# NIH-NEI/oct-image-segmentation-models

Hardware: AMD Instinct MI355X
Metric: B-scans/sec (train step), 256x512 3-class U-Net (higher is better)
Workload: dtype f32; 1 GPU; configs[1]: train step (fwd+Dice-macro+bwd+allreduce+Adam), per-GPU batch 32, 256x512x1, 3-class, pool_layers=4, start_neurons=8, random-init weights; global_batch=32, parallelism=dp1, allreduce=none

## Files before the change

oct-image-segmentation-models_amd/csrc/kernels_bx.hpp:

```cpp
#pragma once
#include <type_traits>

#include "kernels_bwd.hpp"
#include "kernels_igemm.hpp"

namespace oct {

typedef __bf16 bf16x8 __attribute__((ext_vector_type(8)));

__device__ __forceinline__ uint32_t pk_bf16(float a, float b) {
    return __builtin_bit_cast(uint32_t, __builtin_convertvector(f32x2_hw{a, b}, bf16x2_hw));
}

__device__ __forceinline__ void touch_raw(float4& v) { asm volatile("" : "+v"(v.x), "+v"(v.y), "+v"(v.z), "+v"(v.w)); }
__device__ __forceinline__ void touch_raw(uint2& v) { asm volatile("" : "+v"(v.x), "+v"(v.y)); }

__device__ __forceinline__ void act8(float (&v)[8], const float (&fa)[8], const float (&fb)[8], float lo, bool in) {
    const float cl = in ? lo : 0.f, ch = in ? 3.0e38f : 0.f;
#pragma unroll
    for (int i = 0; i < 8; i += 2) {
        const f32x2_hw y = __builtin_elementwise_fma(f32x2_hw{fa[i], fa[i + 1]}, f32x2_hw{v[i], v[i + 1]}, f32x2_hw{fb[i], fb[i + 1]});
        v[i] = __builtin_amdgcn_fmed3f(y[0], cl, ch); v[i + 1] = __builtin_amdgcn_fmed3f(y[1], cl, ch);
    }
}
// ... 360 lines not shown
                    }
            }
        }
    };
    constexpr int EPN = EPI == EPI_MASK ? 4 * MB : (EPI == EPI_FWD ? MB : 0), EPF = (EPN + NTHR - 1) / NTHR;
    float epi_pf[EPF > 0 ? EPF : 1];
    auto load_epi = [&]() {
#pragma unroll
        for (int i = 0; i < EPF; ++i) {
            const int e = tid + i * NTHR;
            float v = 0.f;
            if constexpr (EPI == EPI_FWD) { if (e < MB && m0 + e < A.Mout) v = A.bias[A.m_off + m0 + e]; }
            else if constexpr (EPI == EPI_MASK) { if (e < 4 * MB && m0 + e % MB < A.Mout) v = A.bnin[(e / MB) * A.Mout + m0 + e % MB]; }
            epi_pf[i] = v;
        }
    };
    int g = 0;
#if defined(BX_DBG) && (BX_DBG == 6 || BX_DBG == 7)
    const int nch_run = 0;
    if constexpr (NW == 4) load_zraw();
    load_epi();
#if BX_DBG == 7
    if (A.Cin > 0) return;
#endif
#else
    const int nch_run = nch;
#endif
    for (int c = 0; c < nch_run; ++c) {
#pragma unroll
        for (int ky = 0; ky < KH; ++ky, ++g) {
            const bool last_row = ky == KH - 1, more = c + 1 < nch;
            if (last_row && !more) {
                if constexpr (NW == 4) load_zraw();
                load_epi();
            }
            if (last_row && more) {
#pragma unroll
                for (int k = 0; k < NSLOT; ++k) {
                    touch_raw(pin[k][0]); touch_raw(pin[k][1]);
                    if constexpr (GB) { touch_raw(pz[k][0]); touch_raw(pz[k][1]); }
                }
                if constexpr (NIMG == 2) begin_store((c + 1) * 16);
            }
#if !(defined(BX_DBG) && BX_DBG == 5)
            if (!last_row) dma_slab(c, ky + 1, (g + 1) & 1);
            else if (more) dma_slab(c + 1, 0, (g + 1) & 1);
#endif
            if (ky == 0 && more) load_in((c + 1) * 16);
            if constexpr (NIMG == 2) {
                if (last_row && more) sweep_row(ky, g & 1, c & 1, std::true_type{}, (c + 1) & 1);
                else sweep_row(ky, g & 1, c & 1, std::false_type{}, 0);
            } else {
                sweep_row(ky, g & 1, 0, std::false_type{}, 0);
                if (last_row && more) {
                    begin_store((c + 1) * 16);
                    __syncthreads();
#pragma unroll
                    for (int k = 0; k < NSLOT; ++k) store_slot(k, 0);
                }
            }
            asm volatile("s_waitcnt vmcnt(0)" ::: "memory");
#if !(defined(BX_DBG) && BX_DBG == 1)
            __syncthreads();
#endif
        }
    }
#if defined(BX_DBG) && BX_DBG == 1
    __syncthreads();
#endif

    float* const epi = reinterpret_cast<float*>(WTs);
    float* const red = reinterpret_cast<float*>(WTs + EPI_B);
    if constexpr (NW != 4) load_zraw();
    if constexpr (EPI != EPI_RAW) {
#pragma unroll
        for (int i = 0; i < EPF; ++i) { const int e = tid + i * NTHR; if (e < EPN) epi[e] = epi_pf[i]; }
    }
    __syncthreads();
    float s1[MTW][ACC], s2[MTW][ACC];
#pragma unroll
    for (int mt = 0; mt < MTW; ++mt)
#pragma unroll
        for (int r = 0; r < ACC; ++r) { s1[mt][r] = 0.f; s2[mt][r] = 0.f; }
#pragma unroll
    for (int nt = 0; nt < NTW; ++nt) {
        const int y = y0 + wave * NTW + nt, x = x0 + j;
        const bool pvalid = y < A.Ho && x < A.Wo;
        const size_t pix = pvalid ? ((size_t)b * A.Ho + y) * A.Wo + x : 0;
#pragma unroll
        for (int mt = 0; mt < MTW; ++mt) {
#pragma unroll
            for (int q = 0; q < QUADS; ++q) {
                const int ml = mt * MT + 8 * q + 4 * h, m = m0 + ml;
                const bool valid = pvalid && m < A.Mout;
                float v[4] = {acc[mt][nt][4 * q], acc[mt][nt][4 * q + 1], acc[mt][nt][4 * q + 2], acc[mt][nt][4 * q + 3]};
                if constexpr (EPI == EPI_FWD) {
                    if (valid) {
                        const float4 bs = ld4(epi + ml);
                        v[0] += bs.x; v[1] += bs.y; v[2] += bs.z; v[3] += bs.w;
                    }
#pragma unroll
                    for (int k = 0; k < 4; ++k) {
                        const float u = valid ? v[k] : 0.f;
                        s1[mt][4 * q + k] += u; s2[mt][4 * q + k] += u * u;
                    }
                } else if constexpr (EPI == EPI_MASK) {
                    const float4 zq = widen4(zraw[nt][mt][q]);
                    const float zz[4] = {zq.x, zq.y, zq.z, zq.w};
                    const float4 ea = ld4(epi + BN_A * MB + ml), eb = ld4(epi + BN_B * MB + ml);
                    const float4 em = ld4(epi + BN_MEAN * MB + ml), er = ld4(epi + BN_RSTD * MB + ml);
                    const float ka[4] = {ea.x, ea.y, ea.z, ea.w}, kb[4] = {eb.x, eb.y, eb.z, eb.w};
                    const float km[4] = {em.x, em.y, em.z, em.w}, kr[4] = {er.x, er.y, er.z, er.w};
#pragma unroll
                    for (int k = 0; k < 4; ++k) {
                        const int cc = valid ? m + k : 0;
                        const float yv = fmaf(ka[k], zz[k], kb[k]);
                        float gv = v[k];
                        if (A.drop_out) gv *= drop_mul(A.drop, (uint32_t)(pix * A.Mout + cc));
                        gv = (valid && yv > 0.f) ? gv : 0.f;
                        const float xh = (zz[k] - km[k]) * kr[k];
                        v[k] = gv; s1[mt][4 * q + k] += gv; s2[mt][4 * q + k] += gv * xh;
                    }
                }
                if (valid) sta4<AT>(reinterpret_cast<AT*>(A.out) + pix * A.Mout + m, make_float4(v[0], v[1], v[2], v[3]));
            }
        }
    }
    if constexpr (EPI != EPI_RAW) {
        if (A.part) {
#pragma unroll
            for (int mt = 0; mt < MTW; ++mt) {
                subgroup_reduce_rec<ACC, ACC, 16>(s1[mt], lane);
                subgroup_reduce_rec<ACC, ACC, 16>(s2[mt], lane);
                const int ci = sub_chan<ACC, 16>(lane);
                const int mloc = 8 * (ci >> 2) + 4 * h + (ci & 3);
                red[((wave * 2 + 0) * MTW + mt) * MT + mloc] = s1[mt][0];
                red[((wave * 2 + 1) * MTW + mt) * MT + mloc] = s2[mt][0];
            }
            __syncthreads();
            if (tid < 2 * MB) {
                const int stat = tid / MB, ml = tid % MB, mt = ml / MT, mloc = ml % MT;
                float s = 0.f;
#pragma unroll
                for (int w = 0; w < NW; ++w) s += red[((w * 2 + stat) * MTW + mt) * MT + mloc];
                if (m0 + ml < A.Mout)
                    A.part[((size_t)b * A.tiles + tile) * (2 * A.Mout) + (size_t)stat * A.Mout + m0 + ml] = s;
            }
        }
    }
}

typedef __bf16 bf16x4 __attribute__((ext_vector_type(4)));

template <int KH, bool UP, int NS, typename AT, bool DROP = false, bool GB = false>
__global__ __launch_bounds__(kBlock, 1) void conv_dwbx_k(const ConvBwdWArgs A) {
    constexpr int TH = 4, TW = 32, TAPS = KH * KH;
    constexpr int IH = UP ? TH + 1 : TH + KH - 1, IW = UP ? TW + 1 : TW + KH - 1, PT = UP ? 0 : (KH - 1) / 2;
    constexpr int NPX = IH * IW, NPD = TH * TW;
    constexpr int NXS = (NPX * 4 + kBlock - 1) / kBlock, NDS = (NPD * 4) / kBlock;
    constexpr int NPXP = NXS * (kBlock / 4);
    constexpr int XPL = NPXP * 64, DPL = NPD * 64;
    constexpr int BUF_B = NS * (XPL + DPL);
    static_assert((NPD * 4) % kBlock == 0, "dz tile items");
    constexpr int RED_B = TAPS * 4 * 16 * 64 * 4;
    constexpr int SMEM_B = 2 * BUF_B > RED_B ? 2 * BUF_B : RED_B;
    static_assert(SMEM_B >= 4096 * 4 + kBlock * 8 * 4, "bias scratch fits");
    __shared__ __attribute__((aligned(256))) char smem[SMEM_B];

    const int tid = threadIdx.x, lane = tid & 63, wave = __builtin_amdgcn_readfirstlane(tid >> 6);
    const int ci0 = blockIdx.y * 32, co0 = blockIdx.z * 32;
    const int Hs = UP ? A.H >> 1 : A.H, Ws = UP ? A.W >> 1 : A.W;

    const int o8 = 8 * (tid & 3);
    const int cx = ci0 + o8;
    const bool two = (A.flags & F_TWO) && cx >= A.C0;
    const int Cs = two ? A.C1 : A.C0, ccx = two ? cx - A.C0 : cx;
    const AT* __restrict__ xsrc = (two ? reinterpret_cast<const AT*>(A.x1) : reinterpret_cast<const AT*>(A.x0)) + ccx;
    const AT* __restrict__ dsrc = reinterpret_cast<const AT*>(A.dz) + co0 + o8;
    const AT* __restrict__ zsrc = GB ? reinterpret_cast<const AT*>(A.zf) + co0 + o8 : nullptr;
    const bool aff = (A.flags & F_AFF) != 0;
    const float lo = aff ? 0.f : -3.0e38f;
    float fa[8], fb[8];
#pragma unroll
    for (int i = 0; i < 8; ++i) { fa[i] = 1.f; fb[i] = 0.f; }
    if (aff) {
        const float* ab = two ? A.ab1 : A.ab0;
#pragma unroll
        for (int i = 0; i < 8; ++i) { fa[i] = ab[ccx + i]; fb[i] = ab[Cs + ccx + i]; }
    }
    float ga[GB ? 8 : 1], gb[GB ? 8 : 1], gd[GB ? 8 : 1];
    if constexpr (GB) load_gb8(A.bnf, A.Cout, co0 + o8, ga, gb, gd);
    int xly[NXS], xlx[NXS];
#pragma unroll
    for (int k = 0; k < NXS; ++k) {
        const int P = (tid >> 2) + k * (kBlock / 4);
        xly[k] = P < NPX ? P / IW : -1000000; xlx[k] = P % IW;
    }
    struct Regs { typename Raw4<AT>::type x[NXS][2], d[NDS][2], z[GB ? NDS : 1][2]; };
    float bsum[8];
#pragma unroll
    for (int i = 0; i < 8; ++i) bsum[i] = 0.f;

    auto tile_of = [&](int tl, int& b, int& y0, int& x0) {
        b = tl / A.tiles; const int t = tl % A.tiles;
        x0 = (t % A.tiles_x) * TW; y0 = (t / A.tiles_x) * TH;
    };
    struct Geo { int b, y0, x0; };
    auto geo_of = [&](int tl) { Geo g; tile_of(tl, g.b, g.y0, g.x0); return g; };
    auto load_item = [&](int i, const Geo& g, Regs& R) {
        if (i < NXS) {
            const int k = i;
            int gy = g.y0 + xly[k] - PT, gx = g.x0 + xlx[k] - PT;
            gy = gy < 0 ? 0 : (gy >= A.H ? A.H - 1 : gy); gx = gx < 0 ? 0 : (gx >= A.W ? A.W - 1 : gx);
            const int sy = UP ? gy >> 1 : gy, sx = UP ? gx >> 1 : gx;
            const AT* p = xsrc + (((size_t)g.b * Hs + sy) * Ws + sx) * Cs;
            R.x[k][0] = ldraw4<AT>(p); R.x[k][1] = ldraw4<AT>(p + 4);
        } else {
            const int k = i - NXS;
            const int P = (tid >> 2) + k * (kBlock / 4);
            int py = g.y0 + P / TW, px = g.x0 + P % TW;
            py = py >= A.H ? A.H - 1 : py; px = px >= A.W ? A.W - 1 : px;
            const size_t e = (((size_t)g.b * A.H + py) * A.W + px) * A.Cout;
            R.d[k][0] = ldraw4<AT>(dsrc + e); R.d[k][1] = ldraw4<AT>(dsrc + e + 4);
            if constexpr (GB) { R.z[k][0] = ldraw4<AT>(zsrc + e); R.z[k][1] = ldraw4<AT>(zsrc + e + 4); }
        }
    };
    auto store_item = [&](int i, const Geo& g, const Regs& R, int buf, bool live) {
        if (i < NXS) {
            const int k = i;
            const float4 v0 = widen4(R.x[k][0]), v1 = widen4(R.x[k][1]);
            float v[8] = {v0.x, v0.y, v0.z, v0.w, v1.x, v1.y, v1.z, v1.w};
            const int gy = g.y0 + xly[k] - PT, gx = g.x0 + xlx[k] - PT;
            const bool in = gy >= 0 && gy < A.H && gx >= 0 && gx < A.W;
            act8(v, fa, fb, lo, in);
            if constexpr (DROP) {
                const int sy = UP ? gy >> 1 : gy, sx = UP ? gx >> 1 : gx;
                const uint32_t el = (uint32_t)((((size_t)g.b * Hs + sy) * Ws + sx) * Cs + ccx);
#pragma unroll
                for (int e = 0; e < 8; ++e) v[e] = in ? v[e] * drop_mul(A.drop, el + e) : 0.f;
            }
            uint4 pl[NS];
            split8<NS>(v, pl);
            const int P = (tid >> 2) + k * (kBlock / 4);
            char* d = smem + buf * BUF_B + o8 * 2 + P * 64;
#pragma unroll
            for (int p = 0; p < NS; ++p) *reinterpret_cast<uint4*>(d + p * XPL) = pl[p];
        } else {
            const int k = i - NXS;
            const int P = (tid >> 2) + k * (kBlock / 4);
            const bool in = live && g.y0 + P / TW < A.H && g.x0 + P % TW < A.W;
            const float4 v0 = widen4(R.d[k][0]), v1 = widen4(R.d[k][1]);
            float v[8] = {v0.x, v0.y, v0.z, v0.w, v1.x, v1.y, v1.z, v1.w};
            if constexpr (GB) {
                const float4 z0 = widen4(R.z[k][0]), z1 = widen4(R.z[k][1]);
                const float zv[8] = {z0.x, z0.y, z0.z, z0.w, z1.x, z1.y, z1.z, z1.w};
                gb8<AT>(v, zv, ga, gb, gd, in);
#pragma unroll
                for (int e = 0; e < 8; ++e) bsum[e] += v[e];
            } else {
#pragma unroll
                for (int e = 0; e < 8; ++e) { v[e] = in ? v[e] : 0.f; bsum[e] += v[e]; }
            }
            uint4 pl[NS];
            split8<NS>(v, pl);
            char* d = smem + buf * BUF_B + NS * XPL + o8 * 2 + P * 64;
#pragma unroll
            for (int p = 0; p < NS; ++p) *reinterpret_cast<uint4*>(d + p * DPL) = pl[p];
        }
    };
    constexpr int NIT = NXS + NDS;
    auto load = [&](int tl, Regs& R) {
        const Geo g = geo_of(tl);
#pragma unroll
        for (int i = 0; i < NIT; ++i) load_item(i, g, R);
    };
    auto store = [&](int tl, const Regs& R, int buf, bool live) {
        const Geo g = geo_of(tl);
#pragma unroll
        for (int i = 0; i < NIT; ++i) store_item(i, g, R, buf, live);
    };

    f32x16 acc[TAPS];
#pragma unroll
    for (int t = 0; t < TAPS; ++t)
#pragma unroll
        for (int r = 0; r < 16; ++r) acc[t][r] = 0.f;

    const int laneoff = (8 * (lane >> 5) + ((lane & 15) >> 2)) * 64 + (16 * ((lane >> 4) & 1) + 4 * (lane & 3)) * 2;
    auto tr8 = [&](const char* base) -> bf16x8 {
        const bf16x4 lo = __builtin_amdgcn_ds_read_tr16_b64_v4bf16((__attribute__((address_space(3))) bf16x4*)(base));
        const bf16x4 hi = __builtin_amdgcn_ds_read_tr16_b64_v4bf16((__attribute__((address_space(3))) bf16x4*)(base + 4 * 64));
        return bf16x8{lo[0], lo[1], lo[2], lo[3], hi[0], hi[1], hi[2], hi[3]};
    };
    constexpr int KS = TW / 16, STEPS = KS * TAPS;
    auto compute = [&](int buf, auto&& between) {
        const char* Xl = smem + buf * BUF_B + laneoff;
        const char* Dl = smem + buf * BUF_B + NS * XPL + laneoff + (wave * TW) * 64;
        constexpr int DEPTH = 3;
        bf16x8 av[DEPTH][NS], bw[2][NS];
        auto fetch_a = [&](int st, bf16x8 (&f)[NS]) {
            const int ks = st / TAPS, t = st % TAPS, ky = t / KH, kx = t % KH;
#pragma unroll
            for (int p = 0; p < NS; ++p) f[p] = tr8(Xl + p * XPL + ((wave + ky) * IW + ks * 16 + kx) * 64);
        };
        auto fetch_b = [&](int ks, bf16x8 (&f)[NS]) {
#pragma unroll
            for (int p = 0; p < NS; ++p) f[p] = tr8(Dl + p * DPL + ks * 16 * 64);
        };
        __builtin_amdgcn_s_setprio(1);
        fetch_b(0, bw[0]); fetch_a(0, av[0]); fetch_a(1, av[1]);
#pragma unroll
        for (int st = 0; st < STEPS; ++st) {
            if (st + 2 < STEPS) fetch_a(st + 2, av[(st + 2) % DEPTH]);
            if (st % TAPS == TAPS - 2 && st / TAPS + 1 < KS) fetch_b(st / TAPS + 1, bw[(st / TAPS + 1) & 1]);
            const int t = st % TAPS;
            const bf16x8 (&a)[NS] = av[st % DEPTH];
            const bf16x8 (&bv)[NS] = bw[(st / TAPS) & 1];
            f32x16 c = acc[t];
            if constexpr (NS == 3) {
                c = __builtin_amdgcn_mfma_f32_32x32x16_bf16(a[0], bv[2], c, 0, 0, 0);
                c = __builtin_amdgcn_mfma_f32_32x32x16_bf16(a[2], bv[0], c, 0, 0, 0);
                c = __builtin_amdgcn_mfma_f32_32x32x16_bf16(a[1], bv[1], c, 0, 0, 0);
                c = __builtin_amdgcn_mfma_f32_32x32x16_bf16(a[0], bv[1], c, 0, 0, 0);
                c = __builtin_amdgcn_mfma_f32_32x32x16_bf16(a[1], bv[0], c, 0, 0, 0);
            }
            c = __builtin_amdgcn_mfma_f32_32x32x16_bf16(a[0], bv[0], c, 0, 0, 0);
            acc[t] = c;
            between(st);
        }
        __builtin_amdgcn_s_setprio(0);
        constexpr int NPROD = NS == 3 ? 6 : 1, RPF = 2 * NS;
        constexpr int VPS = NS == 3 ? (UP ? 40 : 26) : (UP ? 24 : 14);
        constexpr int WPS = NS;
        __builtin_amdgcn_sched_group_barrier(0x100, 3 * RPF, 0);
#pragma unroll
        for (int st = 0; st < STEPS; ++st) {
            if (st + 2 < STEPS) __builtin_amdgcn_sched_group_barrier(0x100, RPF, 0);
            if (st % TAPS == TAPS - 2 && st / TAPS + 1 < KS) __builtin_amdgcn_sched_group_barrier(0x100, RPF, 0);
            __builtin_amdgcn_sched_group_barrier(0x008, NPROD, 0);
            __builtin_amdgcn_sched_group_barrier(0x002, VPS, 0);
            if (((st + 1) * NIT) / STEPS != (st * NIT) / STEPS) {
                __builtin_amdgcn_sched_group_barrier(0x200, WPS, 0);
                if (GB && (st * NIT) / STEPS >= NXS) __builtin_amdgcn_sched_group_barrier(0x020, 4, 0);
                else __builtin_amdgcn_sched_group_barrier(0x020, 2, 0);
            }
        }
    };

    Regs R;
    const int t0 = blockIdx.x, step = A.npb, tend = A.total_tiles, tlast = tend - 1;
    if (t0 < tend) {
        load(t0, R);
        store(t0, R, 0, true);
        load(t0 + step < tend ? t0 + step : tlast, R);
    }
    __syncthreads();
    int buf = 0;
    for (int tl = t0; tl < tend; tl += step, buf ^= 1) {
        const int t1 = tl + step, t2 = tl + 2 * step;
        const Geo g1 = geo_of(t1 < tend ? t1 : tlast), g2 = geo_of(t2 < tend ? t2 : tlast);
        const bool live = t1 < tend;
        compute(buf, [&](int st) {
#pragma unroll
            for (int i = 0; i < NIT; ++i)
                if (((st + 1) * NIT) / STEPS != (st * NIT) / STEPS && (st * NIT) / STEPS == i) {
                    store_item(i, g1, R, buf ^ 1, live);
                    load_item(i, g2, R);
                }
        });
        __syncthreads();
    }

    float* const red = reinterpret_cast<float*>(smem);
    float4* const red4 = reinterpret_cast<float4*>(smem);
    const size_t wsize = (size_t)TAPS * A.Cin * A.Cout;
    float* out = A.part + (size_t)blockIdx.x * (wsize + A.Cout);
    __syncthreads();
#pragma unroll
    for (int t = 0; t < TAPS; ++t)
#pragma unroll
        for (int q = 0; q < 4; ++q)
            red4[((wave * TAPS + t) * 4 + q) * 64 + lane] = make_float4(acc[t][4 * q], acc[t][4 * q + 1], acc[t][4 * q + 2], acc[t][4 * q + 3]);
    __syncthreads();
#pragma unroll
    for (int t = 0; t < TAPS; ++t) {
        const int q = wave, e = (t * 4 + q) * 64 + lane;
        const float4 w0 = red4[e], w1 = red4[TAPS * 256 + e], w2 = red4[2 * TAPS * 256 + e], w3 = red4[3 * TAPS * 256 + e];
        const float sv[4] = {(w0.x + w1.x) + (w2.x + w3.x), (w0.y + w1.y) + (w2.y + w3.y),
                             (w0.z + w1.z) + (w2.z + w3.z), (w0.w + w1.w) + (w2.w + w3.w)};
        const int col = lane & 31, row0 = 8 * q + 4 * (lane >> 5);
#pragma unroll
        for (int jr = 0; jr < 4; ++jr)
            if (ci0 + row0 + jr < A.Cin && co0 + col < A.Cout)
                out[((size_t)t * A.Cin + ci0 + row0 + jr) * A.Cout + co0 + col] = sv[jr];
    }
    __syncthreads();
    float* const bs = red + 4096;
#pragma unroll
    for (int i = 0; i < 8; ++i) bs[tid * 8 + i] = bsum[i];
    __syncthreads();
    if (tid < 32 && blockIdx.y == 0 && co0 + tid < A.Cout) {
        const int oct = tid >> 3, comp = tid & 7;
        float s = 0.f;
        for (int t = oct; t < kBlock; t += 4) s += bs[t * 8 + comp];
        out[wsize + co0 + tid] = s;
    }
}

struct WbtDesc {
    const float* src; bf16_t* dst;
    int KH, Kc, M, ld, m_off, CT, NS;
    int m2;
    unsigned start, count;
};

static __global__ __launch_bounds__(kBlock) void prep_wbt_k(const WbtDesc* __restrict__ descs, int nd, unsigned total) {
    for (unsigned e = blockIdx.x * kBlock + threadIdx.x; e < total; e += gridDim.x * kBlock) {
        int d = 0;
        while (d + 1 < nd && e >= descs[d + 1].start) ++d;
        const WbtDesc D = descs[d];
        const unsigned r = e - D.start;
        const int kg = r & 3, m = (r >> 2) & 15, g = r >> 6;
        const int taps = D.KH * D.KH, tpm = 32 / D.CT;
        float v[8];
#pragma unroll
        for (int j = 0; j < 8; ++j) {
            const int k32 = kg * 8 + j, c = k32 % D.CT;
            int tap = g * tpm + k32 / D.CT, mg = D.m_off + m;
            bool ok = tap < taps;
            if (D.m2) {
                const int e = tap, ky = e / (D.KH + 1), kx = e % (D.KH + 1) - (m >> 3);
                ok = e < D.KH * (D.KH + 1) && kx >= 0 && kx < D.KH;
                tap = ky * D.KH + kx; mg = D.m_off + (m & 7);
            }
            v[j] = (ok && c < D.Kc && mg < D.M) ? D.src[((size_t)tap * D.Kc + c) * D.ld + mg] : 0.f;
        }
        bf16_t* base = D.dst + ((size_t)g * D.NS * 16 + m) * 32 + kg * 8;
        if (D.NS == 3) {
            uint4 pl[3]; split8<3>(v, pl);
#pragma unroll
            for (int p = 0; p < 3; ++p) *reinterpret_cast<uint4*>(base + (size_t)p * 16 * 32) = pl[p];
        } else {
            uint4 pl[1]; split8<1>(v, pl);
            *reinterpret_cast<uint4*>(base) = pl[0];
        }
    }
}
__host__ inline int wbt_groups(int KH, int CT, bool m2 = false) { const int tpm = 32 / CT; return (KH * (m2 ? KH + 1 : KH) + tpm - 1) / tpm; }
__host__ inline size_t wbt_bytes(int KH, int CT, int NS, bool m2 = false) { return (size_t)wbt_groups(KH, CT, m2) * NS * 16 * 32 * 2; }

template <int KH, int AMODE, int EPI, int CT, int NS, typename AT, bool M2 = false, bool GB = false, bool FDW = false>
__global__ __launch_bounds__(kBlock, FDW ? 2 : (CT == 32 ? 1 : (CT == 16 ? 2 : 3))) void conv_bt_k(const IgemmArgs A) {
    static_assert(!GB || EPI != EPI_FWD, "the BN-backward transform on load belongs to backward-data launches");
    static_assert(!FDW || (GB && CT == 8 && KH == 3 && AMODE == A_NORMAL), "fused backward-weights: 3x3, 8 K channels, transform on load");
    static_assert(!M2 || ((CT == 8 || CT == 16) && AMODE != A_DOWN2), "two-pixel form: 8 or 16 K channels, unit-stride or upsampled input");
    constexpr int TH = 8, TW = 32, TAPS = KH * (M2 ? KH + 1 : KH), TPM = 32 / CT, NG = (TAPS + TPM - 1) / TPM, OCT = CT / 8;
    constexpr int KW = M2 ? KH + 1 : KH;
    constexpr int NTW = M2 ? 2 : 4, ACC = 4, MB = 16;
    constexpr bool SW2 = M2 && AMODE == A_NORMAL;
    constexpr int IH = AMODE == A_NORMAL ? TH + KH - 1 : (AMODE == A_UPF ? TH / 2 + 1 : 2 * TH + 1);
    constexpr int IW = AMODE == A_NORMAL ? TW + KH - 1 : (AMODE == A_UPF ? TW / 2 + 1 : 2 * TW + 1);
    constexpr int NPIX = IH * IW, PPS = kBlock / OCT, NSLOT = (NPIX + PPS - 1) / PPS, NPIXP = NSLOT * PPS;
    constexpr int PIXB = CT * 2, PLANE_B = NPIXP * PIXB, IN_B = NS * PLANE_B;
    constexpr int SWS = OCT == 4 ? 2 : 3;
    auto lds_off = [](int P, int o) {
        if constexpr (SW2) {
            if constexpr (OCT == 1) return (P ^ ((P >> 4) & 1)) * PIXB;
            else return (P ^ ((P >> 3) & 1)) * PIXB + ((o ^ ((P >> 4) & 1)) * 16);
        } else return P * PIXB + ((o ^ ((P >> SWS) & (OCT - 1))) * 16);
    };
    constexpr int XPL = TH * TW * 16, XIMG_B = FDW ? NS * XPL : 0;
    constexpr bool GBL = GB && CT == 16 && EPI == EPI_MASK && !FDW && sizeof(AT) == 4;
    __shared__ __attribute__((aligned(256))) char smem[2 * IN_B + 2 * XIMG_B + (4 * MB + 4 * 2 * MB) * 4 + (GBL ? 3 * CT * 4 : 0)];
    char* const Xs = smem + 2 * IN_B;
    float* const epi = reinterpret_cast<float*>(smem + 2 * IN_B + 2 * XIMG_B);
    float* const red = epi + 4 * MB;
    float* const gbs = red + 4 * 2 * MB;

    const int tid = threadIdx.x, lane = tid & 63, wave = __builtin_amdgcn_readfirstlane(tid >> 6);
    const int px = lane & 15, kg = lane >> 4;

    bf16x8 wa[NG][NS];
    {
        const char* w = reinterpret_cast<const char*>(A.wbt) + px * 64 + kg * 16;
#pragma unroll
        for (int g = 0; g < NG; ++g)
#pragma unroll
            for (int p = 0; p < NS; ++p) wa[g][p] = *reinterpret_cast<const bf16x8*>(w + (g * NS + p) * 16 * 64);
    }
    if constexpr (EPI == EPI_MASK) {
        for (int e = tid; e < 4 * MB; e += kBlock) {
            const int arr = e / MB, m = e % MB;
            epi[e] = m < A.Mout ? A.bnin[arr * A.Mout + m] : 0.f;
        }
    }
    const int m4 = M2 ? 4 * (kg & 1) : 4 * kg, dx = M2 ? kg >> 1 : 0;
    float4 bias = make_float4(0.f, 0.f, 0.f, 0.f);
    if (EPI == EPI_FWD && m4 < A.Mout) bias = ld4(A.bias + A.m_off + m4);

    const int o = tid % OCT, c8 = 8 * o;
    const bool two = (A.flags & F_TWO) && c8 >= A.C0;
    const int Cs = two ? A.C1 : A.C0, ccx = two ? c8 - A.C0 : c8;
    const AT* __restrict__ xsrc = (two ? reinterpret_cast<const AT*>(A.x1) : reinterpret_cast<const AT*>(A.x0)) + ccx;
    const bool aff = (A.flags & F_AFF) != 0;
    const float lo = aff ? 0.f : -3.0e38f;
    float fa[8], fb[8];
#pragma unroll
    for (int i = 0; i < 8; ++i) { fa[i] = 1.f; fb[i] = 0.f; }
    if (aff) {
        const float* ab = two ? A.ab1 : A.ab0;
#pragma unroll
        for (int i = 0; i < 8; ++i) { fa[i] = ab[ccx + i]; fb[i] = ab[Cs + ccx + i]; }
    }
    float fz[GB ? 8 : 1];
    if constexpr (GBL) {
        if (tid < 3 * CT) {
            const int row = tid / CT, c = tid % CT;
            gbs[tid] = c < A.Cin ? A.gb_bn[(row == 0 ? BN_GA : (row == 1 ? BN_GB : BN_GD)) * A.Cin + c] : 0.f;
        }
        __syncthreads();
// ... 277 lines not shown
#pragma unroll
        for (int nt = 0; nt < NTW; ++nt) {
            const bool valid = pvalid[nt];
            float v[4] = {acc[nt][0], acc[nt][1], acc[nt][2], acc[nt][3]};
            if constexpr (EPI == EPI_FWD) {
                v[0] += bias.x; v[1] += bias.y; v[2] += bias.z; v[3] += bias.w;
#pragma unroll
                for (int k = 0; k < 4; ++k) { const float u = valid ? v[k] : 0.f; s1[k] += u; s2[k] += u * u; }
            } else if constexpr (EPI == EPI_MASK) {
                const float4 zw = widen4(zq[nt]);
                const float zz[4] = {zw.x, zw.y, zw.z, zw.w};
                const int ml = m4 < MB ? m4 : 0;
                const float4 ea = ld4(epi + BN_A * MB + ml), eb = ld4(epi + BN_B * MB + ml);
                const float4 em = ld4(epi + BN_MEAN * MB + ml), er = ld4(epi + BN_RSTD * MB + ml);
                const float ka[4] = {ea.x, ea.y, ea.z, ea.w}, kb[4] = {eb.x, eb.y, eb.z, eb.w};
                const float km[4] = {em.x, em.y, em.z, em.w}, kr[4] = {er.x, er.y, er.z, er.w};
#pragma unroll
                for (int k = 0; k < 4; ++k) {
                    const float yv = fmaf(ka[k], zz[k], kb[k]);
                    float gv = v[k];
                    if (A.drop_out) gv *= drop_mul(A.drop, (uint32_t)tbase + (uint32_t)(valid ? ooff[nt] + k : 0));
                    gv = (valid && yv > 0.f) ? gv : 0.f;
                    const float xh = (zz[k] - km[k]) * kr[k];
                    v[k] = gv; s1[k] += gv; s2[k] += gv * xh;
                }
            }
            if (valid) sta4<AT>(reinterpret_cast<AT*>(A.out) + tbase + ooff[nt], make_float4(v[0], v[1], v[2], v[3]));
        }
        cur = nxt;
        __syncthreads();
    }

    if constexpr (EPI != EPI_RAW) {
        if (A.part) {
            subgroup_reduce_rec<ACC, ACC, 8>(s1, lane);
            subgroup_reduce_rec<ACC, ACC, 8>(s2, lane);
            const int ci = sub_chan<ACC, 8>(lane), mloc = 4 * kg + ci;
            red[(wave * 2 + 0) * MB + mloc] = s1[0];
            red[(wave * 2 + 1) * MB + mloc] = s2[0];
            __syncthreads();
            if (tid < 2 * MB) {
                const int stat = tid / MB, ml = tid % MB;
                float s = (red[(0 * 2 + stat) * MB + ml] + red[(1 * 2 + stat) * MB + ml]) +
                          (red[(2 * 2 + stat) * MB + ml] + red[(3 * 2 + stat) * MB + ml]);
                if constexpr (M2) {
                    const int mh = (ml + 8) % MB;
                    s += (red[(0 * 2 + stat) * MB + mh] + red[(1 * 2 + stat) * MB + mh]) +
                         (red[(2 * 2 + stat) * MB + mh] + red[(3 * 2 + stat) * MB + mh]);
                }
                if (ml < A.Mout) part_store(A.part + (size_t)blockIdx.x * (2 * A.Mout) + (size_t)stat * A.Mout + ml, s);
            }
            if (A.fin.counter) finalize_in_launch(A.fin, A.part, gridDim.x, A.Mout, gridDim.x, smem);
        }
    }
    if constexpr (FDW) {
        __syncthreads();
        float* const r4 = reinterpret_cast<float*>(smem);
#pragma unroll
        for (int a = 0; a < 6; ++a)
#pragma unroll
            for (int r = 0; r < 4; ++r) r4[((wave * 6 + a) * 4 + r) * 64 + lane] = dacc[a][r];
        __syncthreads();
        const int wsize = 9 * A.dw_Cin * 8;
        float* const out = A.dw_part + (size_t)blockIdx.x * (wsize + 8);
        for (int e = tid; e < 6 * 4 * 64; e += kBlock) {
            const float sv = (r4[e] + r4[1536 + e]) + (r4[3072 + e] + r4[4608 + e]);
            const int ln = e & 63, r = (e >> 6) & 3, a = e >> 8;
            const int m = 4 * (ln >> 4) + r, n = ln & 15, ky = a >> 1, kb = a & 1, dxn = n >> 3, co = n & 7;
            const int kx = kb == 0 ? 1 - dxn : 2;
            if (m < 8 && !(kb == 1 && dxn == 1)) out[((ky * 3 + kx) * A.dw_Cin + A.dw_ci_off + m) * 8 + co] = sv;
        }
        __syncthreads();
        block_reduce_store<8>(bsum, r4, out + wsize, A.dw_bias ? 8 : 0);
    }
}

template <int KH, bool UP, int CI, int CO, int NS, typename AT, bool DROP = false, bool GB = false>
__global__ __launch_bounds__(kBlock, (CI + CO >= 48) ? 1 : 2) void conv_dwbt_k(const ConvBwdWArgs A) {
    constexpr int TH = 4, TW = 32, TAPS = KH * KH;
    constexpr int IH = UP ? TH + 1 : TH + KH - 1, IW = UP ? TW + 1 : TW + KH - 1, PT = UP ? 0 : (KH - 1) / 2;
    constexpr int NPX = IH * IW, NPD = TH * TW;
    constexpr int OX = CI / 8, OD = CO / 8;
    constexpr int PPX = kBlock / OX, NXS = (NPX + 4 + PPX - 1) / PPX, NPXP = NXS * PPX;
    constexpr int PPD = kBlock / OD, NDS = (NPD + (CO == 8 ? 1 : 0) + PPD - 1) / PPD, NPDP = NDS * PPD;
    constexpr int XPB = CI * 2, DPB = CO * 2;
    constexpr int XPL = NPXP * XPB, DPL = NPDP * DPB, BUF_B = NS * (XPL + DPL);
    constexpr int MTX = CI == 8 ? (KH + 1) / 2 : KH * (CI / 16);
    constexpr int MTILES = KH * MTX, NTILES = CO == 32 ? 2 : 1, NACC = MTILES * NTILES;
    constexpr int RED_B = 4 * 256 * 4;
    constexpr int SMEM_B = 2 * BUF_B > RED_B + kBlock * 8 * 4 ? 2 * BUF_B : RED_B + kBlock * 8 * 4;
    __shared__ __attribute__((aligned(256))) char smem[SMEM_B];

    const int tid = threadIdx.x, lane = tid & 63, wave = __builtin_amdgcn_readfirstlane(tid >> 6);
    const int Hs = UP ? A.H >> 1 : A.H, Ws = UP ? A.W >> 1 : A.W;

    const int ox = tid % OX, cx = 8 * ox;
    const bool two = (A.flags & F_TWO) && cx >= A.C0;
    const int Cs = two ? A.C1 : A.C0, ccx = two ? cx - A.C0 : cx;
    const AT* __restrict__ xsrc = (two ? reinterpret_cast<const AT*>(A.x1) : reinterpret_cast<const AT*>(A.x0)) + ccx;
    const int od = tid % OD;
    const AT* __restrict__ dsrc = reinterpret_cast<const AT*>(A.dz) + 8 * od;
    const AT* __restrict__ zsrc = GB ? reinterpret_cast<const AT*>(A.zf) + 8 * od : nullptr;
    const bool aff = (A.flags & F_AFF) != 0;
    const float lo = aff ? 0.f : -3.0e38f;
    float fa[8], fb[8];
#pragma unroll
    for (int i = 0; i < 8; ++i) { fa[i] = 1.f; fb[i] = 0.f; }
    if (aff) {
        const float* ab = two ? A.ab1 : A.ab0;
#pragma unroll
        for (int i = 0; i < 8; ++i) { fa[i] = ab[ccx + i]; fb[i] = ab[Cs + ccx + i]; }
    }
    float ga[GB ? 8 : 1], gb[GB ? 8 : 1], gd[GB ? 8 : 1];
    if constexpr (GB) load_gb8(A.bnf, A.Cout, 8 * od, ga, gb, gd);
    int xly[NXS], xlx[NXS];
#pragma unroll
    for (int k = 0; k < NXS; ++k) {
        const int P = tid / OX + k * PPX;
        xly[k] = P < NPX ? P / IW : -1000000; xlx[k] = P % IW;
    }
    struct Regs { typename Raw4<AT>::type x[NXS][2], d[NDS][2], z[GB ? NDS : 1][2]; };
    float bsum[8];
#pragma unroll
    for (int i = 0; i < 8; ++i) bsum[i] = 0.f;

    auto tile_of = [&](int tl, int& b, int& y0, int& x0) {
        b = tl / A.tiles; const int t = tl % A.tiles;
        x0 = (t % A.tiles_x) * TW; y0 = (t / A.tiles_x) * TH;
    };
    struct Geo { int b, y0, x0; };
    auto geo_of = [&](int tl) { Geo g; tile_of(tl, g.b, g.y0, g.x0); return g; };
    constexpr int NIT = NXS + NDS;
    auto load_item = [&](int i, const Geo& g, Regs& R) {
        if (i < NXS) {
            const int k = i;
            int gy = g.y0 + xly[k] - PT, gx = g.x0 + xlx[k] - PT;
            gy = gy < 0 ? 0 : (gy >= A.H ? A.H - 1 : gy); gx = gx < 0 ? 0 : (gx >= A.W ? A.W - 1 : gx);
            const int sy = UP ? gy >> 1 : gy, sx = UP ? gx >> 1 : gx;
            const AT* p = xsrc + (((size_t)g.b * Hs + sy) * Ws + sx) * Cs;
            R.x[k][0] = ldraw4<AT>(p); R.x[k][1] = ldraw4<AT>(p + 4);
        } else {
            const int k = i - NXS;
            const int P = tid / OD + k * PPD;
            int py = g.y0 + P / TW, px = g.x0 + P % TW;
            py = py >= A.H ? A.H - 1 : py; px = px >= A.W ? A.W - 1 : px;
            const size_t e = (((size_t)g.b * A.H + py) * A.W + px) * A.Cout;
            R.d[k][0] = ldraw4<AT>(dsrc + e); R.d[k][1] = ldraw4<AT>(dsrc + e + 4);
            if constexpr (GB) { R.z[k][0] = ldraw4<AT>(zsrc + e); R.z[k][1] = ldraw4<AT>(zsrc + e + 4); }
        }
    };
    auto store_item = [&](int i, const Geo& g, const Regs& R, int buf, bool live) {
        if (i < NXS) {
            const int k = i;
            const float4 v0 = widen4(R.x[k][0]), v1 = widen4(R.x[k][1]);
            float v[8] = {v0.x, v0.y, v0.z, v0.w, v1.x, v1.y, v1.z, v1.w};
            const int gy = g.y0 + xly[k] - PT, gx = g.x0 + xlx[k] - PT;
            const bool in = gy >= 0 && gy < A.H && gx >= 0 && gx < A.W;
            act8(v, fa, fb, lo, in);
            if constexpr (DROP) {
                const int sy = UP ? gy >> 1 : gy, sx = UP ? gx >> 1 : gx;
                const uint32_t el = (uint32_t)((((size_t)g.b * Hs + sy) * Ws + sx) * Cs + ccx);
#pragma unroll
                for (int e = 0; e < 8; ++e) v[e] = in ? v[e] * drop_mul(A.drop, el + e) : 0.f;
            }
            uint4 pl[NS];
            split8<NS>(v, pl);
            const int P = tid / OX + k * PPX;
            char* d = smem + buf * BUF_B + cx * 2 + P * XPB;
#pragma unroll
            for (int p = 0; p < NS; ++p) *reinterpret_cast<uint4*>(d + p * XPL) = pl[p];
        } else {
            const int k = i - NXS;
            const int P = tid / OD + k * PPD;
            const bool in = live && P < NPD && g.y0 + P / TW < A.H && g.x0 + P % TW < A.W;
            const float4 v0 = widen4(R.d[k][0]), v1 = widen4(R.d[k][1]);
            float v[8] = {v0.x, v0.y, v0.z, v0.w, v1.x, v1.y, v1.z, v1.w};
            if constexpr (GB) {
                const float4 z0 = widen4(R.z[k][0]), z1 = widen4(R.z[k][1]);
                const float zv[8] = {z0.x, z0.y, z0.z, z0.w, z1.x, z1.y, z1.z, z1.w};
                gb8<AT>(v, zv, ga, gb, gd, in);
#pragma unroll
                for (int e = 0; e < 8; ++e) bsum[e] += v[e];
            } else {
#pragma unroll
                for (int e = 0; e < 8; ++e) { v[e] = in ? v[e] : 0.f; bsum[e] += v[e]; }
            }
            uint4 pl[NS];
            split8<NS>(v, pl);
            char* d = smem + buf * BUF_B + NS * XPL + od * 16 + P * DPB;
#pragma unroll
            for (int p = 0; p < NS; ++p) *reinterpret_cast<uint4*>(d + p * DPL) = pl[p];
        }
    };
    auto load = [&](int tl, Regs& R) {
        const Geo g = geo_of(tl);
#pragma unroll
        for (int i = 0; i < NIT; ++i) load_item(i, g, R);
    };
    auto store = [&](int tl, const Regs& R, int buf, bool live) {
        const Geo g = geo_of(tl);
#pragma unroll
        for (int i = 0; i < NIT; ++i) store_item(i, g, R, buf, live);
    };

    f32x4 acc[NACC];
#pragma unroll
    for (int t = 0; t < NACC; ++t) acc[t] = f32x4{0.f, 0.f, 0.f, 0.f};

    const int kgq = 8 * (lane >> 4) + ((lane & 15) >> 2), p4 = 4 * (lane & 3);
    const int xlane = kgq * XPB + p4 * 2, dlane = kgq * DPB + p4 * 2;
    auto trx = [&](const char* base, int pitch) -> bf16x8 {
        const bf16x4 lo4 = __builtin_amdgcn_ds_read_tr16_b64_v4bf16((__attribute__((address_space(3))) bf16x4*)(base));
        const bf16x4 hi4 = __builtin_amdgcn_ds_read_tr16_b64_v4bf16((__attribute__((address_space(3))) bf16x4*)(base + 4 * pitch));
        return bf16x8{lo4[0], lo4[1], lo4[2], lo4[3], hi4[0], hi4[1], hi4[2], hi4[3]};
    };
    auto compute = [&](int buf, auto&& between) {
        const char* Xl = smem + buf * BUF_B + xlane;
        const char* Dl = smem + buf * BUF_B + NS * XPL + dlane + (wave * TW) * DPB;
        constexpr int DEPTH = 3;
        bf16x8 bv[NTILES][NS], av[DEPTH][NS];
        auto fetch_a = [&](int mt, bf16x8 (&f)[NS]) {
            const int ky = mt / MTX, mx = mt % MTX;
            const int kx = CI == 8 ? 2 * mx : mx / (CI / 16), cb = CI == 8 ? 0 : (mx % (CI / 16)) * 16;
#pragma unroll
            for (int p = 0; p < NS; ++p) f[p] = trx(Xl + p * XPL + ((wave + ky) * IW + kx) * XPB + cb * 2, XPB);
        };
#pragma unroll
        for (int nt = 0; nt < NTILES; ++nt)
#pragma unroll
            for (int p = 0; p < NS; ++p) bv[nt][p] = trx(Dl + p * DPL + nt * 32, DPB);
        fetch_a(0, av[0]);
        if (MTILES > 1) fetch_a(1, av[1]);
#pragma unroll
        for (int mt = 0; mt < MTILES; ++mt) {
            if (mt + 2 < MTILES) fetch_a(mt + 2, av[(mt + 2) % DEPTH]);
            const bf16x8 (&a)[NS] = av[mt % DEPTH];
#pragma unroll
            for (int nt = 0; nt < NTILES; ++nt) {
                f32x4 c = acc[mt * NTILES + nt];
                if constexpr (NS == 3) {
                    c = __builtin_amdgcn_mfma_f32_16x16x32_bf16(a[0], bv[nt][2], c, 0, 0, 0);
                    c = __builtin_amdgcn_mfma_f32_16x16x32_bf16(a[2], bv[nt][0], c, 0, 0, 0);
                    c = __builtin_amdgcn_mfma_f32_16x16x32_bf16(a[1], bv[nt][1], c, 0, 0, 0);
                    c = __builtin_amdgcn_mfma_f32_16x16x32_bf16(a[0], bv[nt][1], c, 0, 0, 0);
                    c = __builtin_amdgcn_mfma_f32_16x16x32_bf16(a[1], bv[nt][0], c, 0, 0, 0);
                }
                c = __builtin_amdgcn_mfma_f32_16x16x32_bf16(a[0], bv[nt][0], c, 0, 0, 0);
                acc[mt * NTILES + nt] = c;
            }
            between(mt);
        }
        constexpr int NPROD = (NS == 3 ? 6 : 1) * NTILES, RPF = 2 * NS;
        constexpr int VPS = (NIT * (NS == 3 ? 60 : 36) + MTILES - 1) / MTILES, IPS = (NIT + MTILES - 1) / MTILES;
        __builtin_amdgcn_sched_group_barrier(0x100, (NTILES + (MTILES > 1 ? 2 : 1)) * RPF, 0);
#pragma unroll
        for (int mt = 0; mt < MTILES; ++mt) {
            if (mt + 2 < MTILES) __builtin_amdgcn_sched_group_barrier(0x100, RPF, 0);
            __builtin_amdgcn_sched_group_barrier(0x008, NPROD, 0);
            __builtin_amdgcn_sched_group_barrier(0x002, VPS, 0);
            if (((mt + 1) * NIT) / MTILES != (mt * NIT) / MTILES) {
                __builtin_amdgcn_sched_group_barrier(0x200, NS * IPS, 0);
                __builtin_amdgcn_sched_group_barrier(0x020, (GB ? 4 : 2) * IPS, 0);
            }
        }
    };

    Regs R;
    const int t0 = blockIdx.x, step = A.npb, tend = A.total_tiles, tlast = tend - 1;
    if (t0 < tend) {
        load(t0, R);
        store(t0, R, 0, true);
        load(t0 + step < tend ? t0 + step : tlast, R);
    }
    __syncthreads();
    int buf = 0;
    for (int tl = t0; tl < tend; tl += step, buf ^= 1) {
        const int t1 = tl + step, t2 = tl + 2 * step;
        const Geo g1 = geo_of(t1 < tend ? t1 : tlast), g2 = geo_of(t2 < tend ? t2 : tlast);
        const bool live = t1 < tend;
        compute(buf, [&](int mt) {
#pragma unroll
            for (int i = 0; i < NIT; ++i)
                if (i >= (mt * NIT) / MTILES && i < ((mt + 1) * NIT) / MTILES) {
                    store_item(i, g1, R, buf ^ 1, live);
                    load_item(i, g2, R);
                }
        });
        __syncthreads();
    }

    float* const red = reinterpret_cast<float*>(smem);
    const size_t wsize = (size_t)TAPS * A.Cin * A.Cout;
    float* out = A.part + (size_t)blockIdx.x * (wsize + A.Cout);
#pragma unroll
    for (int t = 0; t < NACC; ++t) {
        const int mt = t / NTILES, nt = t % NTILES, ky = mt / MTX, mx = mt % MTX;
        __syncthreads();
#pragma unroll
        for (int r = 0; r < 4; ++r) red[(wave * 4 + r) * 64 + lane] = acc[t][r];
        __syncthreads();
        {
            const int r = tid >> 6, ln = tid & 63;
            const float sv = (red[tid] + red[256 + tid]) + (red[512 + tid] + red[768 + tid]);
            const int col = ln & 15, row = 4 * (ln >> 4) + r;
            int kx, ci;
            if constexpr (CI == 8) { kx = 2 * mx + (row >> 3); ci = row & 7; }
            else { kx = mx / (CI / 16); ci = (mx % (CI / 16)) * 16 + row; }
            const int co = nt * 16 + col;
            if (kx < KH && co < CO)
                out[((size_t)(ky * KH + kx) * A.Cin + ci) * A.Cout + co] = sv;
        }
    }
    __syncthreads();
    float* const bs = red + 1024;
#pragma unroll
    for (int i = 0; i < 8; ++i) bs[tid * 8 + i] = bsum[i];
    __syncthreads();
    if (tid < CO) {
        const int oct = tid >> 3, comp = tid & 7;
        float sv = 0.f;
        for (int t = oct; t < kBlock; t += OD) sv += bs[t * 8 + comp];
        out[wsize + tid] = sv;
    }
}

}
```

Measured before the change: 8414 B-scans/s.

## Load low-res source once for upsampled weight-grad conv and replicate in LDS

For the UP (nearest-upsample) path of the weight-gradient conv kernel, each thread now loads a source pixel from the half-resolution tensor once. It applies the activation and dropout once, then writes the value to four LDS positions (a 2x2 block) in a padded layout. This replaces fetching and processing the full upsampled halo tile, cutting global loads and VALU work roughly fourfold for that operand, at the cost of more LDS stores and a larger padded LDS tile. The schedule-group barrier counts are retuned to match, and compile-time debug switches (DW_DBG) are added that are off by default.

```diff
diff --git a/oct-image-segmentation-models_amd/csrc/kernels_bx.hpp b/oct-image-segmentation-models_amd/csrc/kernels_bx.hpp
--- a/oct-image-segmentation-models_amd/csrc/kernels_bx.hpp
+++ b/oct-image-segmentation-models_amd/csrc/kernels_bx.hpp
@@ -536,13 +536,33 @@
 
 typedef __bf16 bf16x4 __attribute__((ext_vector_type(4)));
 
+#if defined(DW_DBG)
+template <typename T> __device__ inline void dbg_use(const T& v) {
+    uint32_t w[sizeof(T) / 4]; __builtin_memcpy(w, &v, sizeof(T));
+#pragma unroll
+    for (int i = 0; i < (int)(sizeof(T) / 4); ++i) asm volatile("" :: "v"(w[i]));
+}
+template <typename T> __device__ inline void dbg_def(T& v) {
+    uint32_t w[sizeof(T) / 4];
+#pragma unroll
+    for (int i = 0; i < (int)(sizeof(T) / 4); ++i) asm volatile("" : "=v"(w[i]));
+    __builtin_memcpy(&v, w, sizeof(T));
+}
+#define DW_DBG_IS(n) (DW_DBG == (n))
+#else
+#define DW_DBG_IS(n) 0
+#endif
+
 template <int KH, bool UP, int NS, typename AT, bool DROP = false, bool GB = false>
 __global__ __launch_bounds__(kBlock, 1) void conv_dwbx_k(const ConvBwdWArgs A) {
     constexpr int TH = 4, TW = 32, TAPS = KH * KH;
     constexpr int IH = UP ? TH + 1 : TH + KH - 1, IW = UP ? TW + 1 : TW + KH - 1, PT = UP ? 0 : (KH - 1) / 2;
-    constexpr int NPX = IH * IW, NPD = TH * TW;
+    constexpr int LH = TH / 2 + 1, LW = TW / 2 + 1;
+    constexpr int IWP = UP ? IW + 1 : IW, IHP = UP ? IH + 2 : IH;
+    constexpr int NPX = UP ? LH * LW : IH * IW, NPD = TH * TW;
     constexpr int NXS = (NPX * 4 + kBlock - 1) / kBlock, NDS = (NPD * 4) / kBlock;
-    constexpr int NPXP = NXS * (kBlock / 4);
+    constexpr int NPXP = UP ? IHP * IWP : NXS * (kBlock / 4);
+    static_assert(!UP || (kBlock / 4 - NPX) * 2 <= IWP, "UP pad items fit the dump rows");
     constexpr int XPL = NPXP * 64, DPL = NPD * 64;
     constexpr int BUF_B = NS * (XPL + DPL);
     static_assert((NPD * 4) % kBlock == 0, "dz tile items");
@@ -574,11 +594,17 @@
     }
     float ga[GB ? 8 : 1], gb[GB ? 8 : 1], gd[GB ? 8 : 1];
     if constexpr (GB) load_gb8(A.bnf, A.Cout, co0 + o8, ga, gb, gd);
-    int xly[NXS], xlx[NXS];
+    int xly[NXS], xlx[NXS], xpx[NXS];
 #pragma unroll
     for (int k = 0; k < NXS; ++k) {
         const int P = (tid >> 2) + k * (kBlock / 4);
-        xly[k] = P < NPX ? P / IW : -1000000; xlx[k] = P % IW;
+        if constexpr (UP) {
+            xly[k] = P < NPX ? P / LW : -1000000; xlx[k] = P % LW;
+            xpx[k] = P < NPX ? 2 * (P / LW) * IWP + 2 * (P % LW) : (IH + 0) * IWP + 2 * (P - NPX);
+        } else {
+            xly[k] = P < NPX ? P / IW : -1000000; xlx[k] = P % IW;
+            xpx[k] = P;
+        }
     }
     struct Regs { typename Raw4<AT>::type x[NXS][2], d[NDS][2], z[GB ? NDS : 1][2]; };
     float bsum[8];
@@ -594,9 +620,14 @@
     auto load_item = [&](int i, const Geo& g, Regs& R) {
         if (i < NXS) {
             const int k = i;
-            int gy = g.y0 + xly[k] - PT, gx = g.x0 + xlx[k] - PT;
-            gy = gy < 0 ? 0 : (gy >= A.H ? A.H - 1 : gy); gx = gx < 0 ? 0 : (gx >= A.W ? A.W - 1 : gx);
-            const int sy = UP ? gy >> 1 : gy, sx = UP ? gx >> 1 : gx;
+            int sy, sx;
+            if constexpr (UP) {
+                sy = (g.y0 >> 1) + xly[k]; sx = (g.x0 >> 1) + xlx[k];
+                sy = sy < 0 ? 0 : (sy >= Hs ? Hs - 1 : sy); sx = sx >= Ws ? Ws - 1 : sx;
+            } else {
+                int gy = g.y0 + xly[k] - PT, gx = g.x0 + xlx[k] - PT;
+                sy = gy < 0 ? 0 : (gy >= A.H ? A.H - 1 : gy); sx = gx < 0 ? 0 : (gx >= A.W ? A.W - 1 : gx);
+            }
             const AT* p = xsrc + (((size_t)g.b * Hs + sy) * Ws + sx) * Cs;
             R.x[k][0] = ldraw4<AT>(p); R.x[k][1] = ldraw4<AT>(p + 4);
         } else {
@@ -612,27 +643,46 @@
     auto store_item = [&](int i, const Geo& g, const Regs& R, int buf, bool live) {
         if (i < NXS) {
             const int k = i;
+#if DW_DBG_IS(1)
+            uint4 pl[NS];
+            dbg_use(R.x[k]);
+#pragma unroll
+            for (int p = 0; p < NS; ++p) dbg_def(pl[p]);
+#else
             const float4 v0 = widen4(R.x[k][0]), v1 = widen4(R.x[k][1]);
             float v[8] = {v0.x, v0.y, v0.z, v0.w, v1.x, v1.y, v1.z, v1.w};
-            const int gy = g.y0 + xly[k] - PT, gx = g.x0 + xlx[k] - PT;
-            const bool in = gy >= 0 && gy < A.H && gx >= 0 && gx < A.W;
+            const int sy = UP ? (g.y0 >> 1) + xly[k] : g.y0 + xly[k] - PT, sx = UP ? (g.x0 >> 1) + xlx[k] : g.x0 + xlx[k] - PT;
+            const bool in = sy >= 0 && sy < Hs && sx >= 0 && sx < Ws;
             act8(v, fa, fb, lo, in);
             if constexpr (DROP) {
-                const int sy = UP ? gy >> 1 : gy, sx = UP ? gx >> 1 : gx;
                 const uint32_t el = (uint32_t)((((size_t)g.b * Hs + sy) * Ws + sx) * Cs + ccx);
 #pragma unroll
                 for (int e = 0; e < 8; ++e) v[e] = in ? v[e] * drop_mul(A.drop, el + e) : 0.f;
             }
             uint4 pl[NS];
             split8<NS>(v, pl);
-            const int P = (tid >> 2) + k * (kBlock / 4);
-            char* d = smem + buf * BUF_B + o8 * 2 + P * 64;
-#pragma unroll
-            for (int p = 0; p < NS; ++p) *reinterpret_cast<uint4*>(d + p * XPL) = pl[p];
+#endif
+            char* d = smem + buf * BUF_B + o8 * 2 + xpx[k] * 64;
+#pragma unroll
+            for (int p = 0; p < NS; ++p) {
+                *reinterpret_cast<uint4*>(d + p * XPL) = pl[p];
+                if constexpr (UP) {
+                    *reinterpret_cast<uint4*>(d + p * XPL + 64) = pl[p];
+                    *reinterpret_cast<uint4*>(d + p * XPL + IWP * 64) = pl[p];
+                    *reinterpret_cast<uint4*>(d + p * XPL + IWP * 64 + 64) = pl[p];
+                }
+            }
         } else {
             const int k = i - NXS;
             const int P = (tid >> 2) + k * (kBlock / 4);
             const bool in = live && g.y0 + P / TW < A.H && g.x0 + P % TW < A.W;
+#if DW_DBG_IS(1)
+            uint4 pl[NS];
+            dbg_use(R.d[k]);
+            if constexpr (GB) dbg_use(R.z[k]);
+#pragma unroll
+            for (int p = 0; p < NS; ++p) dbg_def(pl[p]);
+#else
             const float4 v0 = widen4(R.d[k][0]), v1 = widen4(R.d[k][1]);
             float v[8] = {v0.x, v0.y, v0.z, v0.w, v1.x, v1.y, v1.z, v1.w};
             if constexpr (GB) {
@@ -647,6 +697,7 @@
             }
             uint4 pl[NS];
             split8<NS>(v, pl);
+#endif
             char* d = smem + buf * BUF_B + NS * XPL + o8 * 2 + P * 64;
 #pragma unroll
             for (int p = 0; p < NS; ++p) *reinterpret_cast<uint4*>(d + p * DPL) = pl[p];
@@ -672,6 +723,9 @@
 
     const int laneoff = (8 * (lane >> 5) + ((lane & 15) >> 2)) * 64 + (16 * ((lane >> 4) & 1) + 4 * (lane & 3)) * 2;
     auto tr8 = [&](const char* base) -> bf16x8 {
+#if DW_DBG_IS(3)
+        bf16x8 r; dbg_def(r); return r;
+#endif
         const bf16x4 lo = __builtin_amdgcn_ds_read_tr16_b64_v4bf16((__attribute__((address_space(3))) bf16x4*)(base));
         const bf16x4 hi = __builtin_amdgcn_ds_read_tr16_b64_v4bf16((__attribute__((address_space(3))) bf16x4*)(base + 4 * 64));
         return bf16x8{lo[0], lo[1], lo[2], lo[3], hi[0], hi[1], hi[2], hi[3]};
@@ -685,7 +739,7 @@
         auto fetch_a = [&](int st, bf16x8 (&f)[NS]) {
             const int ks = st / TAPS, t = st % TAPS, ky = t / KH, kx = t % KH;
 #pragma unroll
-            for (int p = 0; p < NS; ++p) f[p] = tr8(Xl + p * XPL + ((wave + ky) * IW + ks * 16 + kx) * 64);
+            for (int p = 0; p < NS; ++p) f[p] = tr8(Xl + p * XPL + ((wave + ky) * IWP + ks * 16 + kx) * 64);
         };
         auto fetch_b = [&](int ks, bf16x8 (&f)[NS]) {
 #pragma unroll
@@ -700,6 +754,9 @@
             const int t = st % TAPS;
             const bf16x8 (&a)[NS] = av[st % DEPTH];
             const bf16x8 (&bv)[NS] = bw[(st / TAPS) & 1];
+#if DW_DBG_IS(4)
+            dbg_use(a); dbg_use(bv);
+#else
             f32x16 c = acc[t];
             if constexpr (NS == 3) {
                 c = __builtin_amdgcn_mfma_f32_32x32x16_bf16(a[0], bv[2], c, 0, 0, 0);
@@ -710,12 +767,13 @@
             }
             c = __builtin_amdgcn_mfma_f32_32x32x16_bf16(a[0], bv[0], c, 0, 0, 0);
             acc[t] = c;
+#endif
             between(st);
         }
         __builtin_amdgcn_s_setprio(0);
         constexpr int NPROD = NS == 3 ? 6 : 1, RPF = 2 * NS;
-        constexpr int VPS = NS == 3 ? (UP ? 40 : 26) : (UP ? 24 : 14);
-        constexpr int WPS = NS;
+        constexpr int VPS = NS == 3 ? (UP ? 30 : 26) : 14;
+        constexpr int XWPS = UP ? 4 * NS : NS, WPS = NS;
         __builtin_amdgcn_sched_group_barrier(0x100, 3 * RPF, 0);
 #pragma unroll
         for (int st = 0; st < STEPS; ++st) {
@@ -724,7 +782,8 @@
             __builtin_amdgcn_sched_group_barrier(0x008, NPROD, 0);
             __builtin_amdgcn_sched_group_barrier(0x002, VPS, 0);
             if (((st + 1) * NIT) / STEPS != (st * NIT) / STEPS) {
-                __builtin_amdgcn_sched_group_barrier(0x200, WPS, 0);
+                if ((st * NIT) / STEPS < NXS) __builtin_amdgcn_sched_group_barrier(0x200, XWPS, 0);
+                else __builtin_amdgcn_sched_group_barrier(0x200, WPS, 0);
                 if (GB && (st * NIT) / STEPS >= NXS) __builtin_amdgcn_sched_group_barrier(0x020, 4, 0);
                 else __builtin_amdgcn_sched_group_barrier(0x020, 2, 0);
             }
@@ -749,7 +808,11 @@
             for (int i = 0; i < NIT; ++i)
                 if (((st + 1) * NIT) / STEPS != (st * NIT) / STEPS && (st * NIT) / STEPS == i) {
                     store_item(i, g1, R, buf ^ 1, live);
+#if DW_DBG_IS(2)
+                    dbg_def(R);
+#else
                     load_item(i, g2, R);
+#endif
                 }
         });
         __syncthreads();
@@ -1333,6 +1396,12 @@
     auto store_item = [&](int i, const Geo& g, const Regs& R, int buf, bool live) {
         if (i < NXS) {
             const int k = i;
+#if DW_DBG_IS(1)
+            uint4 pl[NS];
+            dbg_use(R.x[k]);
+#pragma unroll
+            for (int p = 0; p < NS; ++p) dbg_def(pl[p]);
+#else
             const float4 v0 = widen4(R.x[k][0]), v1 = widen4(R.x[k][1]);
             float v[8] = {v0.x, v0.y, v0.z, v0.w, v1.x, v1.y, v1.z, v1.w};
             const int gy = g.y0 + xly[k] - PT, gx = g.x0 + xlx[k] - PT;
@@ -1346,6 +1415,7 @@
             }
             uint4 pl[NS];
             split8<NS>(v, pl);
+#endif
             const int P = tid / OX + k * PPX;
             char* d = smem + buf * BUF_B + cx * 2 + P * XPB;
 #pragma unroll
@@ -1354,6 +1424,13 @@
             const int k = i - NXS;
             const int P = tid / OD + k * PPD;
             const bool in = live && P < NPD && g.y0 + P / TW < A.H && g.x0 + P % TW < A.W;
+#if DW_DBG_IS(1)
+            uint4 pl[NS];
+            dbg_use(R.d[k]);
+            if constexpr (GB) dbg_use(R.z[k]);
+#pragma unroll
+            for (int p = 0; p < NS; ++p) dbg_def(pl[p]);
+#else
             const float4 v0 = widen4(R.d[k][0]), v1 = widen4(R.d[k][1]);
             float v[8] = {v0.x, v0.y, v0.z, v0.w, v1.x, v1.y, v1.z, v1.w};
             if constexpr (GB) {
@@ -1368,6 +1445,7 @@
             }
             uint4 pl[NS];
             split8<NS>(v, pl);
+#endif
             char* d = smem + buf * BUF_B + NS * XPL + od * 16 + P * DPB;
 #pragma unroll
             for (int p = 0; p < NS; ++p) *reinterpret_cast<uint4*>(d + p * DPL) = pl[p];
@@ -1391,6 +1469,9 @@
     const int kgq = 8 * (lane >> 4) + ((lane & 15) >> 2), p4 = 4 * (lane & 3);
     const int xlane = kgq * XPB + p4 * 2, dlane = kgq * DPB + p4 * 2;
     auto trx = [&](const char* base, int pitch) -> bf16x8 {
+#if DW_DBG_IS(3)
+        bf16x8 r; dbg_def(r); return r;
+#endif
         const bf16x4 lo4 = __builtin_amdgcn_ds_read_tr16_b64_v4bf16((__attribute__((address_space(3))) bf16x4*)(base));
         const bf16x4 hi4 = __builtin_amdgcn_ds_read_tr16_b64_v4bf16((__attribute__((address_space(3))) bf16x4*)(base + 4 * pitch));
         return bf16x8{lo4[0], lo4[1], lo4[2], lo4[3], hi4[0], hi4[1], hi4[2], hi4[3]};
@@ -1418,6 +1499,9 @@
             const bf16x8 (&a)[NS] = av[mt % DEPTH];
 #pragma unroll
             for (int nt = 0; nt < NTILES; ++nt) {
+#if DW_DBG_IS(4)
+                dbg_use(a); dbg_use(bv[nt]);
+#else
                 f32x4 c = acc[mt * NTILES + nt];
                 if constexpr (NS == 3) {
                     c = __builtin_amdgcn_mfma_f32_16x16x32_bf16(a[0], bv[nt][2], c, 0, 0, 0);
@@ -1428,6 +1512,7 @@
                 }
                 c = __builtin_amdgcn_mfma_f32_16x16x32_bf16(a[0], bv[nt][0], c, 0, 0, 0);
                 acc[mt * NTILES + nt] = c;
+#endif
             }
             between(mt);
         }
@@ -1464,7 +1549,11 @@
             for (int i = 0; i < NIT; ++i)
                 if (i >= (mt * NIT) / MTILES && i < ((mt + 1) * NIT) / MTILES) {
                     store_item(i, g1, R, buf ^ 1, live);
+#if DW_DBG_IS(2)
+                    dbg_def(R);
+#else
                     load_item(i, g2, R);
+#endif
                 }
         });
         __syncthreads();
```

New measurement: 8474 B-scans/s (median of 6 runs). Within noise of the previous version (+0.7%).
